# Priceincoding/nebula

Hardware: AMD Instinct MI355X
Metric: GTEPS for GO 3 STEPS on RMAT-26 at 1/2/4/8 GPUs; % of HBM roofline (higher is better)
Workload: dtype int64; 1 GPU; GO 3 STEPS FROM 64 seeds OVER follow WHERE follow.weight > 499 YIELD DISTINCT follow._dst; RMAT-26 ef16; vertices=32803048, edges_after_collapse=1060378721, edges_scanned_per_query=1545132647, parallelism=1 GPU

## Files before the change

nebula_amd/csrc/snapshot.hip:

```cpp
#include <climits>

#include <rocprim/device/device_merge.hpp>
#include <rocprim/device/device_radix_sort.hpp>
#include <rocprim/device/device_reduce.hpp>
#include <rocprim/device/device_scan.hpp>
#include <rocprim/device/device_select.hpp>
#include <rocprim/iterator/counting_iterator.hpp>

#include <algorithm>
#include <numeric>

#include "device_common.h"
#include "engine.h"
#include "qpred.h"
#include "query_common.h"

namespace nbg {

constexpr int kMaxFields = 64;
struct SchemaDev {
  int32_t nfields;
  int32_t types[kMaxFields];
};

// ... 1283 lines not shown
    case 4: k_gather_w<int32_t><<<g, 256, 0, c.stream>>>(static_cast<const int32_t*>(in), perm, static_cast<int32_t*>(out), m); break;
    default: k_gather_w<int64_t><<<g, 256, 0, c.stream>>>(static_cast<const int64_t*>(in), perm, static_cast<int64_t*>(out), m);
  }
}
static bool copy_prop(const PropCol& p) {
  bool intlike = p.type == NBG_T_INT || p.type == NBG_T_VID || p.type == NBG_T_TIMESTAMP || p.type == NBG_T_BOOL;
  return intlike && !p.present.p;
}


__global__ void k_live_bounds(const int64_t* trp, const uint32_t* odeg, int64_t n, unsigned long long* out) {
  unsigned long long a = 0, b = 0;
  for (int64_t i = blockIdx.x * int64_t(blockDim.x) + threadIdx.x; i < n; i += int64_t(gridDim.x) * blockDim.x)
    if (trp[i + 1] > trp[i]) {
      a = (unsigned long long)(i + 1);
      if (odeg[i]) b = (unsigned long long)(i + 1);
    }
  for (int o = 32; o > 0; o >>= 1) {
    a = max(a, (unsigned long long)__shfl_xor((long long)a, o));
    b = max(b, (unsigned long long)__shfl_xor((long long)b, o));
  }
  if ((threadIdx.x & 63) == 0) {
    if (a) atomicMax(out, a);
    if (b) atomicMax(out + 1, b);
  }
}
__global__ void k_odeg8(const uint32_t* deg, int64_t n, uint8_t* d8) {
  for (int64_t i = blockIdx.x * int64_t(blockDim.x) + threadIdx.x; i < n; i += int64_t(gridDim.x) * blockDim.x)
    d8[i] = uint8_t(min(deg[i], 255u));
}
__global__ void k_out_deg(const int64_t* row_ptr, const uint8_t* row_ok, int64_t n, uint32_t* deg,
                          unsigned int* maxd) {
  unsigned int m = 0;
  for (int64_t i = blockIdx.x * int64_t(blockDim.x) + threadIdx.x; i < n; i += int64_t(gridDim.x) * blockDim.x) {
    uint32_t d = uint32_t(row_ptr[i + 1] - row_ptr[i]);
    if (row_ok && !row_ok[i]) d = 0;
    deg[i] = d;
    m = d > m ? d : m;
  }
  if (maxd) atomicMax(maxd, m);
}
__global__ void k_hub_key(const int32_t* tsrc, int64_t m, const uint32_t* gdeg, uint32_t maxd, uint32_t* key) {
  for (int64_t i = blockIdx.x * int64_t(blockDim.x) + threadIdx.x; i < m; i += int64_t(gridDim.x) * blockDim.x)
    key[i] = maxd - gdeg[tsrc[i]];
}
__global__ void k_gather_u32(const uint32_t* in, const uint32_t* perm, uint32_t* out, int64_t m) {
  for (int64_t i = blockIdx.x * int64_t(blockDim.x) + threadIdx.x; i < m; i += int64_t(gridDim.x) * blockDim.x)
    out[i] = in[perm[i]];
}
__global__ void k_minmax_w(const void* data, int w, int64_t m, long long* mm) {
  long long lo = LLONG_MAX, hi = LLONG_MIN;
  for (int64_t i = blockIdx.x * int64_t(blockDim.x) + threadIdx.x; i < m; i += int64_t(gridDim.x) * blockDim.x) {
    long long v = w == 1 ? static_cast<const int8_t*>(data)[i]
                : w == 2 ? static_cast<const int16_t*>(data)[i]
                : w == 4 ? static_cast<const int32_t*>(data)[i]
                         : static_cast<const int64_t*>(data)[i];
    lo = v < lo ? v : lo;
    hi = v > hi ? v : hi;
  }
  for (int o = 32; o > 0; o >>= 1) {
    const long long a = __shfl_xor(lo, o), b = __shfl_xor(hi, o);
    lo = a < lo ? a : lo;
    hi = b > hi ? b : hi;
  }
  if ((threadIdx.x & 63) == 0) {
    atomicMin(mm, lo);
    atomicMax(mm + 1, hi);
  }
}
__global__ void k_pack_col(const int32_t* col, const void* data, int w, int64_t m, int64_t vmin, uint64_t range,
                           int gbits, int qbits, int32_t* out) {
  for (int64_t i = blockIdx.x * int64_t(blockDim.x) + threadIdx.x; i < m; i += int64_t(gridDim.x) * blockDim.x) {
    const int64_t v = w == 1 ? static_cast<const int8_t*>(data)[i]
                    : w == 2 ? static_cast<const int16_t*>(data)[i]
                    : w == 4 ? static_cast<const int32_t*>(data)[i]
                             : static_cast<const int64_t*>(data)[i];
    out[i] = int32_t((q_bucket(v, vmin, range, qbits) << gbits) | uint32_t(col[i]));
  }
}
template <typename T>
__global__ void k_build_pair(const int64_t* trp, const T* src, int64_t n, T* lo, T* hi, T none) {
  for (int64_t d = blockIdx.x * int64_t(blockDim.x) + threadIdx.x; d < n; d += int64_t(gridDim.x) * blockDim.x) {
    const int64_t b = trp[d], e = trp[d + 1];
#pragma unroll
    for (int q = 0; q < 4; q++) (q < 2 ? lo : hi)[size_t(d) * 2 + (q & 1)] = b + q < e ? src[b + q] : none;
  }
}

__global__ void k_tile_wide(const int64_t* trp, int64_t n, uint32_t* wide) {
  const int lane = threadIdx.x & 63;
  for (int64_t b = blockIdx.x * int64_t(blockDim.x) + threadIdx.x - lane; b < n; b += int64_t(gridDim.x) * blockDim.x) {
    const int64_t d = b + lane;
    const bool w = d < n && trp[d + 1] - trp[d] >= 3;
    const int64_t t = b >> 7;
    if (__ballot(w) != 0ull && lane == 0) atomicOr(wide + (t >> 5), 1u << (uint32_t(t) & 31u));
  }
}

__global__ void k_build_rec(const int64_t* trp, const int32_t* src, int64_t n, uint4* rec) {
  for (int64_t d = blockIdx.x * int64_t(blockDim.x) + threadIdx.x; d < n; d += int64_t(gridDim.x) * blockDim.x) {
    const int64_t b = trp[d], e = trp[d + 1];
    const uint64_t deg = uint64_t(e - b) < 65535u ? uint64_t(e - b) : 65535u;
    uint32_t w[16];
    w[0] = uint32_t(uint64_t(b));
    w[1] = uint32_t(uint64_t(b) >> 32) | uint32_t(deg << 16);
#pragma unroll
    for (int k = 0; k < kRecEntries; k++) w[2 + k] = b + k < e ? uint32_t(src[b + k]) : 0xffffffffu;
#pragma unroll
    for (int j = 0; j < 4; j++) rec[size_t(d) * 4 + j] = make_uint4(w[4 * j], w[4 * j + 1], w[4 * j + 2], w[4 * j + 3]);
  }
}

static void build_transpose(Ctx& c, EdgeSpace& es) {
  Csr& o = es.out;
  Csr& t = es.tr;
  const int64_t m = o.nnz;
  const int64_t lo = c.owned_lo(), hi = c.owned_hi();
  const int64_t n_own = hi - lo;
  const int G = c.world;
  auto nbits = [](int64_t x) {
    int b = 1;
    while ((int64_t(1) << b) < std::max<int64_t>(x, 2)) b++;
    return b;
  };
  const int64_t n_pad = (n_own + 127) / 128 * 128;
  es.odeg.alloc(size_t(n_pad + 1) * 4);
  NBG_HIP(hipMemsetAsync(es.odeg.p, 0, size_t(n_pad + 1) * 4, c.stream));
  DevBuf gdeg, dmax;
  dmax.alloc(16);
  NBG_HIP(hipMemsetAsync(dmax.p, 0, 16, c.stream));
  k_out_deg<<<grid_for(n_own), 256, 0, c.stream>>>(o.row_ptr.as<int64_t>(), o.row_ok.as<uint8_t>(), n_own,
                                                  es.odeg.as<uint32_t>(), dmax.as<unsigned int>());
  es.odeg8.alloc(size_t(n_pad + 64));
  k_odeg8<<<grid_for(n_pad + 1), 256, 0, c.stream>>>(es.odeg.as<uint32_t>(), n_pad + 1, es.odeg8.as<uint8_t>());
  const uint32_t* gdegp = es.odeg.as<uint32_t>();
  if (G > 1) {
    gdeg.alloc(size_t(c.n_global + 1) * 4);
    std::vector<size_t> rb(static_cast<size_t>(G)), ro(static_cast<size_t>(G));
    for (int p = 0; p < G; p++) {
      rb[size_t(p)] = size_t(c.base[size_t(p) + 1] - c.base[size_t(p)]) * 4;
      ro[size_t(p)] = size_t(c.base[size_t(p)]) * 4;
    }
    comm_allgatherv_bytes(c, es.odeg.p, size_t(n_own) * 4, gdeg.p, rb.data(), ro.data());
    gdegp = gdeg.as<uint32_t>();
  }
  uint32_t maxd = 0;
  NBG_HIP(hipMemcpyAsync(&maxd, dmax.p, 4, hipMemcpyDeviceToHost, c.stream));
  NBG_HIP(hipStreamSynchronize(c.stream));
  es.max_odeg = int64_t(maxd);
  if (G > 1) maxd = UINT32_MAX;
  DevBuf tdst, tsrc;
  int64_t R = 0;
  std::vector<const PropCol*> cp;
  for (const PropCol& p : o.props) cp.push_back(copy_prop(p) ? &p : nullptr);
  std::vector<DevBuf> rprops(o.props.size());
  {
    DevBuf esrc;
    esrc.alloc(size_t(m + 1) * 4);
    if (m) k_edge_src<<<grid_for(o.n_rows), 256, 0, c.stream>>>(o.row_ptr.as<int64_t>(), o.n_rows, esrc.as<int32_t>());
    if (G == 1) {
      R = m;
      tsrc = std::move(esrc);
      tdst.alloc(size_t(m + 1) * 4);
      if (m) NBG_HIP(hipMemcpyAsync(tdst.p, o.col.p, size_t(m) * 4, hipMemcpyDeviceToDevice, c.stream));
    } else {
      DevBuf keysB, iota, perm;
      keysB.alloc(size_t(m + 1) * 4);
      iota.alloc(size_t(m + 1) * 4);
      perm.alloc(size_t(m + 1) * 4);
      if (m) {
        k_iota_u32<<<grid_for(m), 256, 0, c.stream>>>(iota.as<uint32_t>(), m);
        radix_pairs<uint32_t, uint32_t>(c, o.col.as<uint32_t>(), keysB.as<uint32_t>(), iota.as<uint32_t>(),
                                       perm.as<uint32_t>(), m, nbits(c.n_global));
      }
      iota.release();
      DevBuf dbase, dcut;
      dbase.alloc(size_t(G + 1) * 8);
      dcut.alloc(size_t(G + 1) * 8);
// ... 57 lines not shown
  for (const PropCol& p : o.props) {
    PropCol q;
    q.name = p.name;
    q.type = p.type;
    q.width = p.width;
    t.props.push_back(std::move(q));
  }
  t.row_ptr.alloc(size_t(t.n_rows + 1) * 8);
  t.col.alloc(size_t(R) * 4 + 64);
  DevBuf perm;
  perm.alloc(size_t(R + 1) * 4);
  if (R) {
    DevBuf key, keyS, iota, perm1;
    key.alloc(size_t(R) * 4);
    keyS.alloc(size_t(R) * 4);
    iota.alloc(size_t(R) * 4);
    perm1.alloc(size_t(R) * 4);
    k_hub_key<<<grid_for(R), 256, 0, c.stream>>>(tsrc.as<int32_t>(), R, gdegp, maxd, key.as<uint32_t>());
    k_iota_u32<<<grid_for(R), 256, 0, c.stream>>>(iota.as<uint32_t>(), R);
    radix_pairs<uint32_t, uint32_t>(c, key.as<uint32_t>(), keyS.as<uint32_t>(), iota.as<uint32_t>(),
                                   perm1.as<uint32_t>(), R, G > 1 ? 32 : nbits(int64_t(maxd) + 1));
    iota.release();
    k_gather_u32<<<grid_for(R), 256, 0, c.stream>>>(tdst.as<uint32_t>(), perm1.as<uint32_t>(), key.as<uint32_t>(), R);
    radix_pairs<uint32_t, uint32_t>(c, key.as<uint32_t>(), keyS.as<uint32_t>(), perm1.as<uint32_t>(),
                                   perm.as<uint32_t>(), R, nbits(n_own));
    k_gather_w<int32_t><<<grid_for(R), 256, 0, c.stream>>>(tsrc.as<int32_t>(), perm.as<uint32_t>(), t.col.as<int32_t>(), R);
    rowptr_from_sorted(c, keyS.as<uint32_t>(), R, t.n_rows, t.row_ptr.as<int64_t>());
  } else {
    NBG_HIP(hipMemsetAsync(t.row_ptr.p, 0, size_t(t.n_rows + 1) * 8, c.stream));
  }
  tsrc.release();
  tdst.release();
  for (size_t f = 0; f < o.props.size(); f++) {
    if (!cp[f]) continue;
    int w = cp[f]->width;
    t.props[f].data.alloc(size_t(R) * size_t(w) + 16);
    const void* src = G == 1 ? cp[f]->data.p : rprops[f].p;
    if (R) gather_width(c, src, perm.as<uint32_t>(), t.props[f].data.p, R, w);
    rprops[f].release();
  }
  if (G == 1) {
    es.t_eid = std::move(perm);
    es.has_t_eid = true;
  } else {
    es.has_t_eid = false;
  }
  for (int h = 0; h < 2; h++) es.pair_col[h].release();
  es.tile_wide.release();
  es.q_field = -1;
  es.q_gbits = es.q_bits = 0;
  es.tcol_q.release();
  if (R > 0) {
    int gb = 1;
    while ((int64_t(1) << gb) <= c.n_global) gb++;
    const int qb = std::min(8, 31 - gb);
    int f = -1;
    for (size_t i = 0; i < t.props.size() && f < 0; i++)
      if (t.props[i].data.p) f = int(i);
    if (qb >= 3 && f >= 0) {
      const PropCol& pc = t.props[size_t(f)];
      DevBuf mm;
      mm.alloc(16);
      const long long init[2] = {LLONG_MAX, LLONG_MIN};
      NBG_HIP(hipMemcpyAsync(mm.p, init, 16, hipMemcpyHostToDevice, c.stream));
      k_minmax_w<<<grid_for(R), 256, 0, c.stream>>>(pc.data.p, pc.width, R, mm.as<long long>());
      long long h[2];
      NBG_HIP(hipMemcpyAsync(h, mm.p, 16, hipMemcpyDeviceToHost, c.stream));
      NBG_HIP(hipStreamSynchronize(c.stream));
      es.q_field = f;
      es.q_gbits = gb;
      es.q_bits = qb;
      es.q_min = h[0];
      es.q_range = uint64_t(h[1]) - uint64_t(h[0]) + 1;
      es.tcol_q.alloc(size_t(R) * 4 + 64);
      k_pack_col<<<grid_for(R), 256, 0, c.stream>>>(t.col.as<int32_t>(), pc.data.p, pc.width, R, es.q_min, es.q_range,
                                                   gb, qb, es.tcol_q.as<int32_t>());
      NBG_HIP(hipGetLastError());
    }
  }
  {
    const int64_t n_pad = (n_own + 127) / 128 * 128;
    for (int h = 0; h < 2; h++) {
      es.pair_col[h].alloc(size_t(n_pad) * 8 + 16);
      NBG_HIP(hipMemsetAsync(es.pair_col[h].as<uint8_t>() + size_t(n_own) * 8, 0xff, size_t(n_pad - n_own) * 8 + 16,
                             c.stream));
    }
    const int32_t* src_col = es.q_field >= 0 ? es.tcol_q.as<int32_t>() : t.col.as<int32_t>();
    if (n_own)
      k_build_pair<int32_t><<<grid_for(n_own), 256, 0, c.stream>>>(t.row_ptr.as<int64_t>(), src_col, n_own,
                                                                   es.pair_col[0].as<int32_t>(),
                                                                   es.pair_col[1].as<int32_t>(), -1);
    const int64_t nt = n_pad / 128;
    es.tile_wide.alloc(size_t(nt / 32 + 2) * 4);
    NBG_HIP(hipMemsetAsync(es.tile_wide.p, 0, size_t(nt / 32 + 2) * 4, c.stream));
    if (n_own)
      k_tile_wide<<<grid_for(n_own), 256, 0, c.stream>>>(t.row_ptr.as<int64_t>(), n_own, es.tile_wide.as<uint32_t>());
  }
  {
    DevBuf lb;
    lb.alloc(16);
    NBG_HIP(hipMemsetAsync(lb.p, 0, 16, c.stream));
    if (n_own)
      k_live_bounds<<<grid_for(n_own), 256, 0, c.stream>>>(t.row_ptr.as<int64_t>(), es.odeg.as<uint32_t>(), n_own,
                                                           lb.as<unsigned long long>());
    unsigned long long h[2] = {0, 0};
    NBG_HIP(hipMemcpyAsync(h, lb.p, 16, hipMemcpyDeviceToHost, c.stream));
    NBG_HIP(hipStreamSynchronize(c.stream));
    es.bu_in_tiles = int64_t((h[0] + 127) / 128);
    es.bu_both_tiles = int64_t((h[1] + 127) / 128);
  }
  es.brec.release();
  es.brec_rows = 0;
  {
    const int64_t rows = std::min(n_own, es.bu_in_tiles * 128);
    const int64_t cap_mb = c.opt("bu_rec_mb", 8192);
    if (rows > 0 && c.opt("bu_rec", 1) != 0 && rows * 64 <= (cap_mb << 20)) {
      es.brec.alloc(size_t(rows) * 64);
      const int32_t* src_col = es.q_field >= 0 ? es.tcol_q.as<int32_t>() : t.col.as<int32_t>();
      k_build_rec<<<grid_for(rows), 256, 0, c.stream>>>(t.row_ptr.as<int64_t>(), src_col, rows, es.brec.as<uint4>());
      NBG_HIP(hipGetLastError());
      es.brec_rows = rows;
    }
  }
  NBG_HIP(hipStreamSynchronize(c.stream));
  NBG_HIP(hipGetLastError());
  es.has_tr = true;
}

__global__ void k_owned_only(const uint64_t* in, int64_t n, int parts, int world, int rank, uint8_t* flag) {
  for (int64_t i = blockIdx.x * int64_t(blockDim.x) + threadIdx.x; i < n; i += int64_t(gridDim.x) * blockDim.x) {
    int64_t v = int64_t(in[i] ^ (1ull << 63));
    flag[i] = dev_owner(v, parts, world) == rank;
  }
}

__global__ void k_count_deg(const int64_t* src, int64_t n, const int64_t* keys, const int32_t* vals, uint64_t mask,
                            bool has_min, int32_t min_idx, unsigned int* deg) {
  for (int64_t i = blockIdx.x * int64_t(blockDim.x) + threadIdx.x; i < n; i += int64_t(gridDim.x) * blockDim.x) {
    const int32_t g = ht_lookup(keys, vals, mask, src[i], has_min, min_idx);
    if (g >= 0) atomicAdd(deg + g, 1u);
  }
}
__global__ void k_class_key(const unsigned int* odeg, const unsigned int* ideg, const uint32_t* idx, int64_t n,
                            uint64_t* key) {
  for (int64_t i = blockIdx.x * int64_t(blockDim.x) + threadIdx.x; i < n; i += int64_t(gridDim.x) * blockDim.x) {
    const int64_t u = idx ? int64_t(idx[i]) : i;
    const uint32_t od = odeg[u];
    if (ideg) {
      const uint32_t id = ideg[u];
      const uint64_t cls = id ? (od ? 0 : 1) : (od ? 2 : 3);
      key[i] = (cls << 34) | (uint64_t(~od) << 2) | uint64_t(3u - min(id, 3u));
    } else {
      key[i] = uint64_t(~od);
    }
  }
}

static void order_by_degree(Ctx& c, DevBuf& owned, int64_t n_owned) {
  if (n_owned <= 1) return;
  int64_t cap = 1024;
  while (cap < 2 * n_owned) cap <<= 1;
  DevBuf keys, vals, vids, deg, dmin;
  keys.alloc(size_t(cap) * 8);
  vals.alloc(size_t(cap) * 4);
  vids.alloc(size_t(n_owned) * 8);
  deg.alloc(size_t(n_owned) * 4);
  dmin.alloc(4);
  fill<int64_t>(c, keys.as<int64_t>(), INT64_MIN, cap);
  int32_t neg = -1;
  NBG_HIP(hipMemcpyAsync(dmin.p, &neg, 4, hipMemcpyHostToDevice, c.stream));
  NBG_HIP(hipMemsetAsync(deg.p, 0, size_t(n_owned) * 4, c.stream));
  k_unflip<<<grid_for(n_owned), 256, 0, c.stream>>>(owned.as<uint64_t>(), vids.as<int64_t>(), n_owned);
  k_ht_insert<<<grid_for(n_owned), 256, 0, c.stream>>>(keys.as<int64_t>(), vals.as<int32_t>(), uint64_t(cap - 1),
                                                       vids.as<int64_t>(), n_owned, 0, dmin.as<int32_t>());
  int32_t min_idx = -1;
  NBG_HIP(hipMemcpyAsync(&min_idx, dmin.p, 4, hipMemcpyDeviceToHost, c.stream));
  NBG_HIP(hipStreamSynchronize(c.stream));
// ... 1078 lines not shown
```

nebula_amd/csrc/traverse.hip:

```cpp
#include <chrono>
#include <rocprim/device/device_radix_sort.hpp>
#include <rocprim/device/device_reduce.hpp>
#include <rocprim/device/device_scan.hpp>
#include <rocprim/device/device_select.hpp>

#include <algorithm>
#include <cmath>
#include <unordered_map>
#include <thread>
#include <type_traits>
#include <initializer_list>

#include "device_common.h"
#include "engine.h"
#include "expr_device.h"
#include "program.h"
#include "qpred.h"
#include "query_common.h"
#include "rows.h"

namespace nbg {

constexpr int kThreads = 256;
constexpr int kItems = 8;
// ... 453 lines not shown
  }
}

struct GateIn {
  const unsigned long long* e = nullptr;
  const unsigned long long* n = nullptr;
  const unsigned long long* pg = nullptr;
  unsigned long long thr = 0;
  const unsigned long long* all = nullptr;
  int world = 1;
  int shards = 1;
};
__device__ inline bool gate_open(const GateIn& gi, unsigned long long* gate) {
  if (gi.e == nullptr && gi.all == nullptr) return gate == nullptr || *gate != 0ull;
  unsigned long long n, e;
  if (gi.all) {
    n = e = 0ull;
    for (int r = 0; r < gi.world; r++) n += gi.all[2 * r], e += gi.all[2 * r + 1];
  } else {
    n = e = 0ull;
    for (int s = 0; s < gi.shards; s++) n += gi.n[size_t(s) * kShardStride], e += gi.e[size_t(s) * kShardStride];
  }
  const bool open = (gi.pg == nullptr || *gi.pg != 0ull) && n > 0ull && e >= gi.thr;
  if (blockIdx.x == 0 && threadIdx.x == 0) {
    __hip_atomic_store(gate, open ? 1ull : 0ull, __ATOMIC_RELAXED, __HIP_MEMORY_SCOPE_AGENT);
    if (gi.all) {
      __hip_atomic_store(gate + (kSpecSumN - kSpecGate), n, __ATOMIC_RELAXED, __HIP_MEMORY_SCOPE_AGENT);
      __hip_atomic_store(gate + (kSpecSumE - kSpecGate), e, __ATOMIC_RELAXED, __HIP_MEMORY_SCOPE_AGENT);
    }
  }
  return open;
}

template <int PK, int U, int HUB, int STATS, int NT = 0, int SKIP = 0>
__global__ __launch_bounds__(1024, 8) void k_bu_lean(const uint2* __restrict__ lo, const uint2* __restrict__ hi,
                                                     int64_t ntiles, int64_t work_tiles,
                                                     const uint32_t* __restrict__ fbits, uint32_t fb_bytes,
                                                     unsigned long long* __restrict__ nbits,
                                                     unsigned long long* __restrict__ pbits,
                                                     const uint32_t* __restrict__ odeg, QArgs q_arg,
                                                     unsigned long long* __restrict__ partials, int cw,
                                                     const uint8_t* __restrict__ odeg8,
                                                     unsigned long long* gate, GateIn gi, int atomic_sums) {
  if (!gate_open(gi, gate)) return;
  __shared__ unsigned long long lds[kSlots * 16];
  extern __shared__ uint32_t s_fb[];
  if (HUB) hub_fill(s_fb, fbits, cw, true);
  const QArgs q = q_sgpr(q_arg);
  constexpr bool FINAL = PK == PK_FAST;
  constexpr int NS = FINAL ? 4 : 2;
  const __amdgpu_buffer_rsrc_t fb_rs =
      __builtin_amdgcn_make_buffer_rsrc(const_cast<uint32_t*>(fbits), 0, int(fb_bytes), 0x00020000);
  const uint32_t gmask = q.gmask, ucw = uint32_t(cw);
  const int lane = threadIdx.x & 63;
  const int64_t wave = (int64_t(blockIdx.x) * blockDim.x + threadIdx.x) >> 6;
  const int64_t nwaves = (int64_t(gridDim.x) * blockDim.x) >> 6;
  uint32_t nglob = 0, nhub = 0;
  unsigned long long nfound = 0, npend = 0, nwords = 0;
  unsigned long long odsum = 0;
  auto prep = [&](uint32_t sw, int k, uint32_t& goff, uint32_t& lidx, uint32_t& pm, uint32_t& um) {
    const uint32_t wi = (sw & gmask) >> 5;
    bool cand = true;
    if (FINAL) {
      const int st = q_test(int32_t(sw), q);
      const bool und = st < 0, pass = st > 0;
      cand = st != 0;
      pm |= pass ? 1u << k : 0u;
      um |= und ? 1u << k : 0u;
    }
    const bool hub = HUB && wi < ucw;
    goff = cand && !hub ? wi * 4u : 0xfffffff0u;
    lidx = cand && hub ? wi : ucw;
    if (STATS) {
      nglob += cand && !hub;
      nhub += cand && hub;
    }
  };
  auto bit = [](uint32_t w, uint32_t sw) -> uint32_t { return __builtin_amdgcn_ubfe(w, sw & 31u, 1u); };
  auto row_of = [&](int64_t t, int h) -> int64_t { return t * 128 + lane + 64 * h; };
  for (int64_t t0 = wave * U; t0 < work_tiles; t0 += nwaves * U) {
    uint2 a[U][2], b[U][2];
    uint32_t od[U][2];
    bool v[U];
#pragma unroll
    for (int u = 0; u < U; u++) {
      v[u] = t0 + u < work_tiles;
      const int64_t r = (v[u] ? t0 + u : t0) * 128 + lane;
#pragma unroll
      for (int h = 0; h < 2; h++) {
        if (NT) {
          const uint64_t x = __builtin_nontemporal_load(reinterpret_cast<const uint64_t*>(lo + r + 64 * h));
          a[u][h] = make_uint2(uint32_t(x), uint32_t(x >> 32));
          if (FINAL) {
            const uint64_t y = __builtin_nontemporal_load(reinterpret_cast<const uint64_t*>(hi + r + 64 * h));
            b[u][h] = make_uint2(uint32_t(y), uint32_t(y >> 32));
          }
          od[u][h] = FINAL ? 1u : uint32_t(__builtin_nontemporal_load(odeg8 + r + 64 * h));
        } else {
          a[u][h] = lo[r + 64 * h];
          if (FINAL) b[u][h] = hi[r + 64 * h];
          od[u][h] = FINAL ? 1u : odeg[r + 64 * h];
        }
      }
    }
    __builtin_amdgcn_sched_barrier(0);
    uint32_t goff[U][2][NS], lidx[U][2][NS], pm[U][2], um[U][2];
#pragma unroll
    for (int u = 0; u < U; u++)
#pragma unroll
      for (int h = 0; h < 2; h++) {
        pm[u][h] = um[u][h] = 0u;
        prep(a[u][h].x, 0, goff[u][h][0], lidx[u][h][0], pm[u][h], um[u][h]);
        prep(a[u][h].y, 1, goff[u][h][1], lidx[u][h][1], pm[u][h], um[u][h]);
        if (FINAL) {
          prep(b[u][h].x, 2, goff[u][h][2], lidx[u][h][2], pm[u][h], um[u][h]);
          prep(b[u][h].y, 3, goff[u][h][3], lidx[u][h][3], pm[u][h], um[u][h]);
        }
      }
    uint32_t lw[U][2][NS], gw[U][2][NS];
    if (HUB) {
#pragma unroll
      for (int u = 0; u < U; u++)
#pragma unroll
        for (int h = 0; h < 2; h++)
#pragma unroll
          for (int k = 0; k < NS; k++) {
            if (SKIP) {
              lw[u][h][k] = 0u;
              if (__ballot(lidx[u][h][k] != ucw)) lw[u][h][k] = s_fb[lidx[u][h][k]];
            } else {
              lw[u][h][k] = s_fb[lidx[u][h][k]];
            }
          }
    }
    bool noprobe[U][2];
#pragma unroll
    for (int u = 0; u < U; u++)
#pragma unroll
      for (int h = 0; h < 2; h++) {
        noprobe[u][h] = false;
        if ((SKIP & 2) && HUB && !FINAL) {
          const uint32_t sw[2] = {a[u][h].x, a[u][h].y};
          bool hf = false;
#pragma unroll
          for (int k = 0; k < NS; k++) hf = hf || bit(lw[u][h][k], sw[k]) != 0u;
          noprobe[u][h] = hf || od[u][h] == 0u;
        }
      }
#pragma unroll
    for (int u = 0; u < U; u++)
#pragma unroll
      for (int h = 0; h < 2; h++)
#pragma unroll
        for (int k = 0; k < NS; k++) {
          if (SKIP) {
            gw[u][h][k] = 0u;
            const uint32_t go = noprobe[u][h] ? 0xfffffff0u : goff[u][h][k];
            if (__ballot(go != 0xfffffff0u)) gw[u][h][k] = __builtin_amdgcn_raw_buffer_load_b32(fb_rs, go, 0, 0);
          } else {
            gw[u][h][k] = __builtin_amdgcn_raw_buffer_load_b32(fb_rs, goff[u][h][k], 0, 0);
          }
        }
    __builtin_amdgcn_sched_barrier(0);
    bool f[U][2], pend[U][2];
#pragma unroll
    for (int u = 0; u < U; u++) {
#pragma unroll
      for (int h = 0; h < 2; h++) {
        const uint32_t sw[4] = {a[u][h].x, a[u][h].y, b[u][h].x, b[u][h].y};
        uint32_t hm = 0u;
#pragma unroll
        for (int k = 0; k < NS; k++) hm |= bit(HUB ? (lw[u][h][k] | gw[u][h][k]) : gw[u][h][k], sw[k]) << k;
        if (FINAL) {
          f[u][h] = (hm & pm[u][h]) != 0u;
          pend[u][h] = v[u] && !f[u][h] && (b[u][h].y != 0xffffffffu || (hm & um[u][h]) != 0u);
        } else {
          f[u][h] = hm != 0u && od[u][h] > 0;
          pend[u][h] = v[u] && hm == 0u && od[u][h] > 0 && a[u][h].y != 0xffffffffu;
        }
      }
      nwords += v[u] ? (FINAL ? 8u : 4u) * 64u : 0u;
    }
    if (!FINAL) {
      bool anyp = false;
#pragma unroll
// ... 20 lines not shown
            prep(b[u][h].x, 0, g2[u][h][0], l2[u][h][0], d0, d1);
            prep(b[u][h].y, 1, g2[u][h][1], l2[u][h][1], d0, d1);
          }
        uint32_t lv[U][2][2], gv[U][2][2];
        if (HUB) {
#pragma unroll
          for (int u = 0; u < U; u++)
#pragma unroll
            for (int h = 0; h < 2; h++)
#pragma unroll
              for (int k = 0; k < 2; k++) lv[u][h][k] = s_fb[l2[u][h][k]];
        }
#pragma unroll
        for (int u = 0; u < U; u++)
#pragma unroll
          for (int h = 0; h < 2; h++)
#pragma unroll
            for (int k = 0; k < 2; k++) gv[u][h][k] = __builtin_amdgcn_raw_buffer_load_b32(fb_rs, g2[u][h][k], 0, 0);
#pragma unroll
        for (int u = 0; u < U; u++)
#pragma unroll
          for (int h = 0; h < 2; h++) {
            const uint32_t w0 = HUB ? (lv[u][h][0] | gv[u][h][0]) : gv[u][h][0];
            const uint32_t w1 = HUB ? (lv[u][h][1] | gv[u][h][1]) : gv[u][h][1];
            const bool g = (bit(w0, b[u][h].x) | bit(w1, b[u][h].y)) != 0u;
            f[u][h] = f[u][h] || (pend[u][h] && g);
            pend[u][h] = pend[u][h] && !g && b[u][h].y != 0xffffffffu;
          }
      } else {
#pragma unroll
        for (int u = 0; u < U; u++) pend[u][0] = pend[u][1] = false;
      }
    }
#pragma unroll
    for (int u = 0; u < U; u++) {
      if (!v[u]) continue;
      const int64_t t = t0 + u;
      unsigned long long f0 = __ballot(f[u][0]), f1 = __ballot(f[u][1]);
      unsigned long long p0 = __ballot(pend[u][0]), p1 = __ballot(pend[u][1]);
      if (SKIP & 4) {
        if (lane < 2) {
          typedef unsigned long long u64x2 __attribute__((ext_vector_type(2)));
          u64x2 vv;
          vv.x = lane ? p0 : f0;
          vv.y = lane ? p1 : f1;
          *reinterpret_cast<u64x2*>((lane ? pbits : nbits) + 2 * t) = vv;
        }
      } else if (lane < 2) {
        nbits[2 * t + lane] = lane ? f1 : f0;
        pbits[2 * t + lane] = lane ? p1 : p0;
      }
      nfound += uint64_t(__popcll(f0) + __popcll(f1));
      npend += uint64_t(__popcll(p0) + __popcll(p1));
      if (!FINAL) {
#pragma unroll
        for (int h = 0; h < 2; h++) {
          uint32_t d = f[u][h] ? od[u][h] : 0u;
          if (NT && d == 255u) d = odeg[row_of(t, h)];
          odsum += uint64_t(d);
        }
      }
    }
  }
  for (int64_t t = work_tiles + wave; t < ntiles; t += nwaves)
    if (lane < 2) {
      nbits[2 * t + lane] = 0ull;
      pbits[2 * t + lane] = 0ull;
    }
  if (lane != 0) nfound = npend = nwords = 0;
  unsigned long long acc64[8] = {nfound, odsum, nwords, npend, 0, 0, nglob, nhub};
  if (atomic_sums) block_add_sums(acc64, 8, lds, partials, atomic_sums);
  else block_store_partials(acc64, 8, lds, partials);
}

constexpr uint32_t kNoProbe = 0x0ffffff0u;
template <int CLS, int NT>
__global__ __launch_bounds__(1024, 8) void k_bu_fin(const uint2* __restrict__ lo, const uint2* __restrict__ hi,
                                                    int64_t ntiles, int64_t work_tiles,
                                                    const uint32_t* __restrict__ fbits,
                                                    unsigned long long* __restrict__ nbits,
                                                    unsigned long long* __restrict__ pbits, FinArgs fa_arg,
                                                    unsigned long long* __restrict__ partials, int cw,
                                                    uint32_t fb_rest, unsigned long long* gate, GateIn gi,
                                                    int atomic_sums, const uint32_t* __restrict__ wide) {
  if (!gate_open(gi, gate)) return;
  extern __shared__ uint32_t s_fb[];
  unsigned long long* lds = reinterpret_cast<unsigned long long*>(s_fb + ((cw + 2) & ~1));
  hub_fill(s_fb, fbits, cw, true);
  const uint32_t clo = __builtin_amdgcn_readfirstlane(fa_arg.clo), cr = __builtin_amdgcn_readfirstlane(fa_arg.cr);
  const uint32_t plo = __builtin_amdgcn_readfirstlane(fa_arg.plo), pr = __builtin_amdgcn_readfirstlane(fa_arg.pr);
  const bool pinv = __builtin_amdgcn_readfirstlane(fa_arg.pinv) != 0;
  const uint32_t bmask = __builtin_amdgcn_readfirstlane(fa_arg.bmask);
  const uint32_t cw4 = __builtin_amdgcn_readfirstlane(uint32_t(cw) * 4u);
  const __amdgpu_buffer_rsrc_t fb_rs = __builtin_amdgcn_make_buffer_rsrc(
      const_cast<uint32_t*>(fbits + cw), 0, int(__builtin_amdgcn_readfirstlane(fb_rest)), 0x00020000);
  typedef const __attribute__((address_space(3))) uint32_t* lds_u32p;
  const int lane = threadIdx.x & 63;
  const int64_t wave =
      int64_t(__builtin_amdgcn_readfirstlane(uint32_t((int64_t(blockIdx.x) * blockDim.x + threadIdx.x) >> 6)));
  const int64_t nwaves = (int64_t(gridDim.x) * blockDim.x) >> 6;
  unsigned long long nfound = 0, npend = 0, nwords = 0;
  auto ld8 = [&](const uint2* p) -> uint2 {
    if (!NT) return *p;
    const uint64_t x = __builtin_nontemporal_load(reinterpret_cast<const uint64_t*>(p));
    return make_uint2(uint32_t(x), uint32_t(x >> 32));
  };
  const uint32_t rest_b = __builtin_amdgcn_readfirstlane(fb_rest);
  auto tile = [&](int64_t t, auto ns_c) {
    constexpr int NS = decltype(ns_c)::value;
    uint32_t sw[2][NS];
    const int64_t r = t * 128 + lane;
#pragma unroll
    for (int h = 0; h < 2; h++) {
      const uint2 a = ld8(lo + r + 64 * h);
      sw[h][0] = a.x, sw[h][1] = a.y;
      if (NS == 4) {
        const uint2 b = ld8(hi + r + 64 * h);
        sw[h][NS - 2] = b.x, sw[h][NS - 1] = b.y;
      }
    }
    __builtin_amdgcn_sched_barrier(0);
    uint32_t ob[2][NS];
#pragma unroll
    for (int h = 0; h < 2; h++)
#pragma unroll
      for (int k = 0; k < NS; k++) {
        const uint32_t w = sw[h][k];
        if (CLS == 1)
          ob[h][k] = ((w >> 3) & bmask) | fin_skip_cls1(w, clo);
        else
          ob[h][k] = fin_candidate(w, clo, cr) ? (w >> 3) & bmask : kNoProbe;
      }
    uint32_t lw[2][NS], gw[2][NS];
#pragma unroll
    for (int h = 0; h < 2; h++)
#pragma unroll
      for (int k = 0; k < NS; k++) lw[h][k] = *(lds_u32p)(size_t(min(ob[h][k], cw4)));
    bool hubf[2] = {false, false};
#pragma unroll
    for (int h = 0; h < 2; h++)
#pragma unroll
      for (int k = 0; k < NS; k++) {
        const uint32_t w = sw[h][k];
        const bool pass = CLS == 1 ? w >= plo : (w - plo <= pr) != pinv;
        hubf[h] = hubf[h] || (__builtin_amdgcn_ubfe(lw[h][k], w, 1u) != 0u && pass);
      }
#pragma unroll
    for (int h = 0; h < 2; h++)
#pragma unroll
      for (int k = 0; k < NS; k++) {
        gw[h][k] = 0u;
        if (__ballot(ob[h][k] - cw4 < rest_b && !hubf[h]))
          gw[h][k] = __builtin_amdgcn_raw_buffer_load_b32(fb_rs, hubf[h] ? 0xfffffff0u : ob[h][k] - cw4, 0, 0);
      }
    __builtin_amdgcn_sched_barrier(0);
    bool f[2], pend[2];
#pragma unroll
    for (int h = 0; h < 2; h++) {
      bool fh = false, ah = false;
#pragma unroll
      for (int k = 0; k < NS; k++) {
        const uint32_t w = sw[h][k];
        const bool hit = __builtin_amdgcn_ubfe(lw[h][k] | gw[h][k], w, 1u) != 0u;
        const bool pass = CLS == 1 ? w >= plo : (w - plo <= pr) != pinv;
        fh = fh || (hit && pass);
        ah = ah || hit;
      }
      f[h] = fh;
      pend[h] = !fh && (ah || (NS == 4 && sw[h][NS - 1] != 0xffffffffu));
    }
    unsigned long long f0 = __ballot(f[0]), f1 = __ballot(f[1]);
    unsigned long long p0 = __ballot(pend[0]), p1 = __ballot(pend[1]);
    if (lane < 2) {
      typedef unsigned long long u64x2 __attribute__((ext_vector_type(2)));
      u64x2 v;
      v.x = lane ? p0 : f0;
      v.y = lane ? p1 : f1;
      *reinterpret_cast<u64x2*>((lane ? pbits : nbits) + 2 * t) = v;
    }
    nfound += uint64_t(__popcll(f0) + __popcll(f1));
    npend += uint64_t(__popcll(p0) + __popcll(p1));
    nwords += uint64_t(2 * NS) * 64u;
  };
  auto wide_word = [&](int64_t t) -> uint32_t {
    if (!wide) return 0xffffffffu;
    return wide[__builtin_amdgcn_readfirstlane(uint32_t(min(t, work_tiles) >> 5))];
  };
  uint32_t ww = wave < work_tiles ? wide_word(wave) : 0u;
  for (int64_t t = wave; t < work_tiles; t += nwaves) {
    const uint32_t wbit = __builtin_amdgcn_readfirstlane((ww >> (uint32_t(t) & 31u)) & 1u);
    __builtin_amdgcn_sched_barrier(0);
    ww = wide_word(t + nwaves);
    if (wbit)
      tile(t, std::integral_constant<int, 4>{});
    else
      tile(t, std::integral_constant<int, 2>{});
  }
  for (int64_t t = work_tiles + wave; t < ntiles; t += nwaves)
    if (lane < 2) {
      nbits[2 * t + lane] = 0ull;
      pbits[2 * t + lane] = 0ull;
    }
  if (lane != 0) nfound = npend = nwords = 0;
  unsigned long long acc64[8] = {nfound, 0, nwords, npend, 0, 0, 0, 0};
  if (atomic_sums) block_add_sums(acc64, 8, lds, partials, atomic_sums);
  else block_store_partials(acc64, 8, lds, partials);
}

constexpr int kLeanChunk = 8;
__device__ inline void load_chunk8(const int32_t* __restrict__ tcol, int64_t a, int64_t re, bool act,
                                   int32_t (&sv)[kLeanChunk]) {
  int4 x = make_int4(-1, -1, -1, -1), y = x;
  if (act) x = *reinterpret_cast<const int4*>(tcol + a);
  if (act && a + 4 < re) y = *reinterpret_cast<const int4*>(tcol + a + 4);
  sv[0] = x.x, sv[1] = x.y, sv[2] = x.z, sv[3] = x.w;
  sv[4] = y.x, sv[5] = y.y, sv[6] = y.z, sv[7] = y.w;
}
template <int PK, int W, int HUB, int REC>
__global__ __launch_bounds__(1024, 4) void k_bu_rest_lean(const unsigned long long* __restrict__ pbits, int64_t n,
                                                          const int64_t* __restrict__ trp,
                                                          const int32_t* __restrict__ tcol,
                                                          const uint32_t* __restrict__ fbits, uint32_t fb_bytes,
                                                          unsigned long long* nbits,
                                                          const uint32_t* __restrict__ odeg, FastArgs fp, QArgs q_arg,
                                                          unsigned long long* partials, int cw, int ru, int rest_from,
                                                          int steps, unsigned long long* dbg,
                                                          const unsigned long long* __restrict__ gate,
                                                          const uint4* __restrict__ rec, int atomic_sums) {
  if (gate && *gate == 0ull) return;
  const QArgs q = q_sgpr(q_arg);
  __shared__ unsigned long long lds[kSlots * 16];
  __shared__ unsigned long long s_found[16][64];
  extern __shared__ uint32_t s_fb[];
  const unsigned long long t_in = wall_clock64();
  if (HUB) hub_fill(s_fb, fbits, cw, false);
  const unsigned long long t_hub = wall_clock64();
  uint32_t d_rows = 0, d_batches = 0, d_steps = 0, d_scan = 0;
  unsigned long long t_scan = 0;
  const __amdgpu_buffer_rsrc_t fb_rs = __builtin_amdgcn_make_buffer_rsrc(
      const_cast<uint32_t*>(fbits), 0, int(__builtin_amdgcn_readfirstlane(fb_bytes)), 0x00020000);
  auto in_front = [&](int32_t g) -> bool {
    const int32_t wi = g >> 5;
    uint32_t w;
    if (HUB && wi < cw) w = s_fb[wi];
    else w = __builtin_amdgcn_raw_buffer_load_b32(fb_rs, wi * 4, 0, 0);
    return (w >> (g & 31)) & 1u;
  };
  uint32_t acc[6] = {0, 0, 0, 0, 0, 0};
  unsigned long long odsum = 0;
  const int lane = threadIdx.x & 63, wv = threadIdx.x >> 6;
  const int64_t nwords = (n + 63) / 64;
  const int64_t wave = (int64_t(blockIdx.x) * blockDim.x + threadIdx.x) >> 6;
  const int64_t nwaves = (int64_t(gridDim.x) * blockDim.x) >> 6;
  for (int64_t cbase = 0; cbase + wave < nwords; cbase += nwaves * 64) {
    const int64_t myw = cbase + int64_t(lane) * nwaves + wave;
    const unsigned long long pw = myw < nwords ? pbits[myw] : 0ull;
    s_found[wv][lane] = 0ull;
    uint32_t total;
    const uint32_t pre = wave_excl_scan(uint32_t(__popcll(pw)), total);
    for (uint32_t k0 = 0; k0 < total; k0 += 64) {
      const uint32_t p = k0 + uint32_t(lane);
      bool pend[1] = {p < total}, found[1] = {false};
      int64_t rb[1] = {0}, re[1] = {0};
      int wsel = 0;
#pragma unroll
      for (int st = 32; st > 0; st >>= 1) {
        const uint32_t pv = __shfl(pre, wsel + st);
        if (wsel + st < 64 && pv <= p) wsel += st;
      }
      const unsigned long long wbits = __shfl((long long)pw, wsel);
      const uint32_t kk = p - __shfl(pre, wsel);
      int bit = 0;
#pragma unroll
      for (int st = 32; st > 0; st >>= 1)
        if (uint32_t(__popcll(wbits & ((1ull << (bit + st)) - 1ull))) <= kk) bit += st;
      const int32_t r = int32_t((cbase + int64_t(wsel) * nwaves + wave) * 64 + bit);
      auto test_chunk = [&](const int32_t(&sv)[kLeanChunk], int64_t base, int64_t lo_e, int64_t hi_e, bool act,
                            bool count) __attribute__((always_inline)) -> bool {
        uint32_t w[kLeanChunk];
// ... 1165 lines not shown
}

static void launch_bits_vids(Ctx& c, const uint32_t* bits, int64_t rows, int64_t lo, void* out,
                             unsigned long long* n_out, const unsigned long long* gate) {
  const int grid = grid_cap((rows + 31) / 32, 1024, 4096);
  k_bits_compact<1, 8, 1><<<grid, 1024, 0, c.stream>>>(bits, rows, lo, c.vid_of.as<int64_t>(), out, n_out, gate);
}

struct BuLaunch {
  size_t ev_first = kNoEvent;
  std::string k0, k1;
  bool rest_rec = false;
  uint64_t od_bytes = 0;
  uint64_t flag_bytes = 0;
};
BuLaunch launch_bu_lean(Ctx& c, EdgeSpace& es, const uint32_t* fb, uint32_t* nbits, const uint32_t* odeg, int pk,
                      const FastArgs& fp, int fcol, unsigned long long* out, bool hop_front,
                      unsigned long long* gate = nullptr, GateIn gi = GateIn{}, bool out_zero = false,
                      int shards = 1) {
  const Csr& tr = es.tr;
  if (pk != PK_NONE && pk != PK_FAST) throw Error(NBG_E_DEVICE, "bottom-up hop with a VM predicate");
  if (!es.pair_col[0].p) throw Error(NBG_E_DEVICE, "bottom-up hop without the quad slab");
  const bool fast = pk == PK_FAST || !odeg;
  QArgs q;
  if (pk == PK_FAST) {
    q = make_qargs(es, c.opt("bu_qpred", 1) != 0 ? pk : PK_NONE, fcol, fp);
  } else {
    q = make_qargs(es, PK_NONE, -1, fp);
    if (fast) q.ulo = q.uhi = INT32_MAX, q.below = q.above = 1;
  }
  const int rest_from = pk == PK_FAST ? 0 : 4;
  pk = fast ? PK_FAST : PK_NONE;
  const int64_t ntiles = (tr.n_rows + 127) / 128;
  const int64_t work = std::min(ntiles, fast ? es.bu_in_tiles : es.bu_both_tiles);
  const int64_t waves = std::max<int64_t>(1, work);
  const int64_t fb_words = (c.n_global + 31) / 32;
  const int64_t hub_cap = std::max<int64_t>(0, c.opt("bu_hub_cap", 36 * 1024));
  const int cw = int(std::min<int64_t>(c.opt(fast ? "bu_lean_lds_kb_final" : "bu_lean_lds_kb", fast ? 72 : 64) * 256,
                                       std::min<int64_t>({fb_words, int64_t(36 * 1024), hub_cap})));
  const int bs = cw > 0 ? 1024 : 256;
  const int grid = int(std::max<int64_t>(
      1, std::min<int64_t>((waves + bs / 64 - 1) / (bs / 64),
                           std::min<int64_t>(cw > 0 ? 512 : 2048, kAggBlocks / 2))));
  const size_t shm = size_t(cw + 1) * 4;
  uint32_t fb_bytes = uint32_t(fb_words * 4);
  if (hop_front && !c.sharded && es.bu_both_tiles > 0)
    fb_bytes = uint32_t(std::min<int64_t>(fb_bytes, (es.bu_both_tiles * 128 + 31) / 32 * 4));
  const int probe_stats = int(c.opt("bu_probe_stats", 0));
  c.ws_pend.ensure(size_t(ntiles * 2 + 2) * 8);
  unsigned long long* pbits = c.ws_pend.as<unsigned long long>();
  const int atomic_sums =
      c.opt("bu_atomic_sums", 1) != 0 && c.opt("bu_rest_dbg", 0) == 0 ? (out_zero ? std::max(shards, 1) : 1) : 0;
  unsigned long long* partials = atomic_sums ? out : c.ws_partials.as<unsigned long long>();
  if (atomic_sums && !out_zero) NBG_HIP(hipMemsetAsync(out, 0, 8 * 8, c.stream));
  auto* nb = reinterpret_cast<unsigned long long*>(nbits);
  const uint2* lo = es.pair_col[0].as<uint2>();
  const uint2* hi = es.pair_col[1].as<uint2>();
  const uint32_t* od = fast ? nullptr : odeg;
  auto go = [&](auto kern) {
    if (shm > 48 * 1024)
      lds_limit(reinterpret_cast<const void*>(kern), shm);
    kern<<<grid, bs, shm, c.stream>>>(lo, hi, ntiles, work, fb, fb_bytes, nb, pbits, od, q, partials, cw,
                                      es.odeg8.as<uint8_t>(), gate, gi, atomic_sums);
  };
  int sel = probe_stats ? 4 + (cw > 0 ? 1 : 0) : (cw > 0 ? 2 : 0);
  if (sel == 2 && (fast || es.odeg8.p)) sel = 8;
#define NBG_LEAN(PKV)                                \
  switch (sel) {                                     \
    case 8: go(k_bu_lean<PKV, 1, 1, 0, 1, 3>); break; \
    case 0: go(k_bu_lean<PKV, 1, 0, 0>); break;      \
    case 2: go(k_bu_lean<PKV, 1, 1, 0>); break;      \
    case 4: go(k_bu_lean<PKV, 1, 0, 1>); break;      \
    default: go(k_bu_lean<PKV, 1, 1, 1>); break;     \
  }
  const bool fin = fast && !probe_stats && c.opt("bu_fin", 1) != 0;
  uint64_t flag_bytes = 0;
  char fin_nm[64] = "";
  if (fin) {
    const FinArgs fa = fin_args(q);
    const bool cls1 = fin_cls1_ok(fa) && c.opt("bu_fin_cls", 1) != 0;
    const size_t fshm = size_t((cw + 2) & ~1) * 4 + size_t(kSlots) * 16 * 8;
    const uint32_t rest = fb_bytes > uint32_t(cw) * 4u ? fb_bytes - uint32_t(cw) * 4u : 0u;
    const int nt = int(c.opt("bu_fin_nt", 1) != 0);
    const uint32_t* wide = c.opt("bu_fin_narrow", 1) != 0 ? es.tile_wide.as<uint32_t>() : nullptr;
    if (wide) flag_bytes = uint64_t(work) / 8;
    auto gof = [&](auto kern) {
      if (fshm > 48 * 1024) lds_limit(reinterpret_cast<const void*>(kern), fshm);
      kern<<<grid, bs, fshm, c.stream>>>(lo, hi, ntiles, work, fb, nb, pbits, fa, partials, cw, rest, gate, gi,
                                         atomic_sums, wide);
    };
    switch ((cls1 ? 1 : 0) | nt << 1) {
      case 0: gof(k_bu_fin<0, 0>); break;
      case 1: gof(k_bu_fin<1, 0>); break;
      case 2: gof(k_bu_fin<0, 1>); break;
      default: gof(k_bu_fin<1, 1>); break;
    }
    snprintf(fin_nm, sizeof fin_nm, "nbg::k_bu_fin<%d, %d>", cls1 ? 1 : 0, nt);
  } else if (fast) {
    NBG_LEAN(PK_FAST)
  } else {
    NBG_LEAN(PK_NONE)
  }
#undef NBG_LEAN
  NBG_HIP(hipGetLastError());
  const size_t ev_first = timing_event(c);
  const int64_t* trp = tr.row_ptr.as<int64_t>();
  const int32_t* tc = q.gbits ? es.tcol_q.as<int32_t>() : tr.col.as<int32_t>();
  const int ru = int(std::max<int64_t>(1, std::min<int64_t>(c.opt("bu_unroll", 1), kRestMax)));
  const int grid2 = 512;
  const int W = fast ? int(fp.width) : 0;
  const int rcw = int(std::min<int64_t>(c.opt(fast ? "bu_rest_lds_kb_final" : "bu_rest_lds_kb", 0) * 256,
                                        std::min<int64_t>({fb_words, int64_t(36 * 1024), hub_cap})));
  const size_t rshm = size_t(std::max(rcw, 1)) * 4;
  const int rsteps = int(std::max<int64_t>(1, c.opt("bu_rest_steps", 4)));
  DevBuf dbg_buf;
  unsigned long long* dbg = nullptr;
  if (c.opt("bu_rest_dbg", 0)) {
    dbg_buf.alloc(size_t(grid2) * 16 * 64);
    NBG_HIP(hipMemsetAsync(dbg_buf.p, 0, size_t(grid2) * 16 * 64, c.stream));
    dbg = dbg_buf.as<unsigned long long>();
  }
  const int64_t rest_rows = std::min(tr.n_rows, work * 128);
  const bool use_rec = es.brec.p && es.brec_rows >= std::min(tr.n_rows, work * 128) && c.opt("bu_rec", 1) != 0;
  const uint4* rec = use_rec ? es.brec.as<uint4>() : nullptr;
  auto rest = [&](auto kern) {
    if (rshm > 48 * 1024)
      lds_limit(reinterpret_cast<const void*>(kern), rshm);
    kern<<<grid2, 1024, rshm, c.stream>>>(pbits, rest_rows, trp, tc, fb, fb_bytes, nb, odeg, fp, q,
                                          atomic_sums ? partials : partials + grid, rcw, ru, rest_from, rsteps, dbg,
                                          gate, rec, atomic_sums);
  };
#define NBG_REST(PKV, WV)                                                 \
  if (rcw > 0) {                                                          \
    if (use_rec) rest(k_bu_rest_lean<PKV, WV, 1, 1>);                     \
    else rest(k_bu_rest_lean<PKV, WV, 1, 0>);                             \
  } else {                                                                \
    if (use_rec) rest(k_bu_rest_lean<PKV, WV, 0, 1>);                     \
    else rest(k_bu_rest_lean<PKV, WV, 0, 0>);                             \
  }
  if (fast) {
    switch (W) {
      case 1: NBG_REST(PK_FAST, 1); break;
      case 2: NBG_REST(PK_FAST, 2); break;
      case 4: NBG_REST(PK_FAST, 4); break;
      default: NBG_REST(PK_FAST, 8); break;
    }
  } else {
    NBG_REST(PK_NONE, 0);
  }
#undef NBG_REST
  NBG_HIP(hipGetLastError());
  if (!atomic_sums) k_reduce_partials<<<1, 1024, 0, c.stream>>>(partials, grid + grid2, out, gate);
  NBG_HIP(hipGetLastError());
  if (dbg) {
    std::vector<unsigned long long> h(size_t(grid2) * 16 * 8);
    NBG_HIP(hipMemcpyAsync(h.data(), dbg, h.size() * 8, hipMemcpyDeviceToHost, c.stream));
    NBG_HIP(hipStreamSynchronize(c.stream));
    if (const char* fn = getenv("NBG_DBG_FILE")) {
      if (FILE* f = fopen(fn, "ab")) {
        const uint64_t hdr[2] = {uint64_t(pk), uint64_t(grid2) * 16};
        fwrite(hdr, 8, 2, f);
        fwrite(h.data(), 8, h.size(), f);
        fclose(f);
      }
    }
  }
  char nm[96];
  if (fin)
    snprintf(nm, sizeof nm, "%s", fin_nm);
  else
    snprintf(nm, sizeof nm, "nbg::k_bu_lean<%d, 1, %d, %d%s>", pk, cw > 0 ? 1 : 0, probe_stats ? 1 : 0,
             sel == 8 ? ", 1, 3" : ", 0, 0");
// ... 1263 lines not shown
```

Baseline: 4131 GTEPS.

## Interleave lo pair columns per tile and add single-slot tier for degree-1 tiles

Changes the lo pair-column layout so slot 0 of both half-tiles is contiguous and slot 1 sits 128 entries later. Tiles whose vertices all have degree at most 1 can then read only the first slot block. A second per-tile flag word (degree >= 2) is added to tile_wide, and the fin kernel dispatches to NS=1, 2 or 4 variants, with NS=1 as the new default. This is meant to cut HBM bytes scanned for low-degree tiles in the bottom-up final step. The cost is twice as much flag metadata, and the lean kernel's loads now use the new layout, which is a consistency risk.

```diff
diff --git a/nebula_amd/csrc/snapshot.hip b/nebula_amd/csrc/snapshot.hip
--- a/nebula_amd/csrc/snapshot.hip
+++ b/nebula_amd/csrc/snapshot.hip
@@ -1389,8 +1389,13 @@
 __global__ void k_build_pair(const int64_t* trp, const T* src, int64_t n, T* lo, T* hi, T none) {
   for (int64_t d = blockIdx.x * int64_t(blockDim.x) + threadIdx.x; d < n; d += int64_t(gridDim.x) * blockDim.x) {
     const int64_t b = trp[d], e = trp[d + 1];
+    const size_t p = size_t(d >> 7) * 256 + size_t(d & 63) * 2 + size_t((d >> 6) & 1);
 #pragma unroll
-    for (int q = 0; q < 4; q++) (q < 2 ? lo : hi)[size_t(d) * 2 + (q & 1)] = b + q < e ? src[b + q] : none;
+    for (int q = 0; q < 4; q++) {
+      const T x = b + q < e ? src[b + q] : none;
+      if (q < 2) lo[p + size_t(q) * 128] = x;
+      else hi[size_t(d) * 2 + (q & 1)] = x;
+    }
   }
 }
 
@@ -1398,9 +1403,13 @@
   const int lane = threadIdx.x & 63;
   for (int64_t b = blockIdx.x * int64_t(blockDim.x) + threadIdx.x - lane; b < n; b += int64_t(gridDim.x) * blockDim.x) {
     const int64_t d = b + lane;
-    const bool w = d < n && trp[d + 1] - trp[d] >= 3;
+    const int64_t deg = d < n ? trp[d + 1] - trp[d] : 0;
     const int64_t t = b >> 7;
-    if (__ballot(w) != 0ull && lane == 0) atomicOr(wide + (t >> 5), 1u << (uint32_t(t) & 31u));
+    const bool w3 = __ballot(deg >= 3) != 0ull, w2 = __ballot(deg >= 2) != 0ull;
+    if (lane == 0) {
+      if (w3) atomicOr(wide + 2 * (t >> 5), 1u << (uint32_t(t) & 31u));
+      if (w2) atomicOr(wide + 2 * (t >> 5) + 1, 1u << (uint32_t(t) & 31u));
+    }
   }
 }
 
@@ -1624,8 +1633,8 @@
     const int64_t n_pad = (n_own + 127) / 128 * 128;
     for (int h = 0; h < 2; h++) {
       es.pair_col[h].alloc(size_t(n_pad) * 8 + 16);
-      NBG_HIP(hipMemsetAsync(es.pair_col[h].as<uint8_t>() + size_t(n_own) * 8, 0xff, size_t(n_pad - n_own) * 8 + 16,
-                             c.stream));
+      const size_t from = h == 0 ? 0 : size_t(n_own) * 8;
+      NBG_HIP(hipMemsetAsync(es.pair_col[h].as<uint8_t>() + from, 0xff, size_t(n_pad) * 8 + 16 - from, c.stream));
     }
     const int32_t* src_col = es.q_field >= 0 ? es.tcol_q.as<int32_t>() : t.col.as<int32_t>();
     if (n_own)
@@ -1633,8 +1642,8 @@
                                                                    es.pair_col[0].as<int32_t>(),
                                                                    es.pair_col[1].as<int32_t>(), -1);
     const int64_t nt = n_pad / 128;
-    es.tile_wide.alloc(size_t(nt / 32 + 2) * 4);
-    NBG_HIP(hipMemsetAsync(es.tile_wide.p, 0, size_t(nt / 32 + 2) * 4, c.stream));
+    es.tile_wide.alloc(size_t(nt / 32 + 2) * 8);
+    NBG_HIP(hipMemsetAsync(es.tile_wide.p, 0, size_t(nt / 32 + 2) * 8, c.stream));
     if (n_own)
       k_tile_wide<<<grid_for(n_own), 256, 0, c.stream>>>(t.row_ptr.as<int64_t>(), n_own, es.tile_wide.as<uint32_t>());
   }
diff --git a/nebula_amd/csrc/traverse.hip b/nebula_amd/csrc/traverse.hip
--- a/nebula_amd/csrc/traverse.hip
+++ b/nebula_amd/csrc/traverse.hip
@@ -559,25 +559,23 @@
     uint2 a[U][2], b[U][2];
     uint32_t od[U][2];
     bool v[U];
+    auto ld8 = [&](const uint2* p) -> uint2 {
+      if (!NT) return *p;
+      const uint64_t x = __builtin_nontemporal_load(reinterpret_cast<const uint64_t*>(p));
+      return make_uint2(uint32_t(x), uint32_t(x >> 32));
+    };
 #pragma unroll
     for (int u = 0; u < U; u++) {
       v[u] = t0 + u < work_tiles;
       const int64_t r = (v[u] ? t0 + u : t0) * 128 + lane;
+      const uint2 s0 = ld8(lo + r), s1 = ld8(lo + r + 64);
+      a[u][0] = make_uint2(s0.x, s1.x);
+      a[u][1] = make_uint2(s0.y, s1.y);
 #pragma unroll
       for (int h = 0; h < 2; h++) {
-        if (NT) {
-          const uint64_t x = __builtin_nontemporal_load(reinterpret_cast<const uint64_t*>(lo + r + 64 * h));
-          a[u][h] = make_uint2(uint32_t(x), uint32_t(x >> 32));
-          if (FINAL) {
-            const uint64_t y = __builtin_nontemporal_load(reinterpret_cast<const uint64_t*>(hi + r + 64 * h));
-            b[u][h] = make_uint2(uint32_t(y), uint32_t(y >> 32));
-          }
-          od[u][h] = FINAL ? 1u : uint32_t(__builtin_nontemporal_load(odeg8 + r + 64 * h));
-        } else {
-          a[u][h] = lo[r + 64 * h];
-          if (FINAL) b[u][h] = hi[r + 64 * h];
-          od[u][h] = FINAL ? 1u : odeg[r + 64 * h];
-        }
+        if (FINAL) b[u][h] = ld8(hi + r + 64 * h);
+        if (NT) od[u][h] = FINAL ? 1u : uint32_t(__builtin_nontemporal_load(odeg8 + r + 64 * h));
+        else od[u][h] = FINAL ? 1u : odeg[r + 64 * h];
       }
     }
     __builtin_amdgcn_sched_barrier(0);
@@ -764,7 +762,8 @@
                                                     unsigned long long* __restrict__ pbits, FinArgs fa_arg,
                                                     unsigned long long* __restrict__ partials, int cw,
                                                     uint32_t fb_rest, unsigned long long* gate, GateIn gi,
-                                                    int atomic_sums, const uint32_t* __restrict__ wide) {
+                                                    int atomic_sums, const uint32_t* __restrict__ wide,
+                                                    int one_slot) {
   if (!gate_open(gi, gate)) return;
   extern __shared__ uint32_t s_fb[];
   unsigned long long* lds = reinterpret_cast<unsigned long long*>(s_fb + ((cw + 2) & ~1));
@@ -792,11 +791,15 @@
     constexpr int NS = decltype(ns_c)::value;
     uint32_t sw[2][NS];
     const int64_t r = t * 128 + lane;
-#pragma unroll
-    for (int h = 0; h < 2; h++) {
-      const uint2 a = ld8(lo + r + 64 * h);
-      sw[h][0] = a.x, sw[h][1] = a.y;
-      if (NS == 4) {
+    const uint2 a = ld8(lo + r);
+    sw[0][0] = a.x, sw[1][0] = a.y;
+    if constexpr (NS >= 2) {
+      const uint2 a1 = ld8(lo + r + 64);
+      sw[0][1] = a1.x, sw[1][1] = a1.y;
+    }
+    if constexpr (NS == 4) {
+#pragma unroll
+      for (int h = 0; h < 2; h++) {
         const uint2 b = ld8(hi + r + 64 * h);
         sw[h][NS - 2] = b.x, sw[h][NS - 1] = b.y;
       }
@@ -864,19 +867,23 @@
     npend += uint64_t(__popcll(p0) + __popcll(p1));
     nwords += uint64_t(2 * NS) * 64u;
   };
-  auto wide_word = [&](int64_t t) -> uint32_t {
-    if (!wide) return 0xffffffffu;
-    return wide[__builtin_amdgcn_readfirstlane(uint32_t(min(t, work_tiles) >> 5))];
+  const uint32_t two_or = one_slot ? 0u : 0xffffffffu;
+  auto wide_word = [&](int64_t t) -> uint2 {
+    if (!wide) return make_uint2(0xffffffffu, 0xffffffffu);
+    return reinterpret_cast<const uint2*>(wide)[__builtin_amdgcn_readfirstlane(uint32_t(min(t, work_tiles) >> 5))];
   };
-  uint32_t ww = wave < work_tiles ? wide_word(wave) : 0u;
+  uint2 ww = wave < work_tiles ? wide_word(wave) : make_uint2(0u, 0u);
   for (int64_t t = wave; t < work_tiles; t += nwaves) {
-    const uint32_t wbit = __builtin_amdgcn_readfirstlane((ww >> (uint32_t(t) & 31u)) & 1u);
+    const uint32_t wbit = __builtin_amdgcn_readfirstlane((ww.x >> (uint32_t(t) & 31u)) & 1u);
+    const uint32_t tbit = __builtin_amdgcn_readfirstlane(((ww.y | two_or) >> (uint32_t(t) & 31u)) & 1u);
     __builtin_amdgcn_sched_barrier(0);
     ww = wide_word(t + nwaves);
     if (wbit)
       tile(t, std::integral_constant<int, 4>{});
+    else if (tbit)
+      tile(t, std::integral_constant<int, 2>{});
     else
-      tile(t, std::integral_constant<int, 2>{});
+      tile(t, std::integral_constant<int, 1>{});
   }
   for (int64_t t = work_tiles + wave; t < ntiles; t += nwaves)
     if (lane < 2) {
@@ -2208,12 +2215,13 @@
     const size_t fshm = size_t((cw + 2) & ~1) * 4 + size_t(kSlots) * 16 * 8;
     const uint32_t rest = fb_bytes > uint32_t(cw) * 4u ? fb_bytes - uint32_t(cw) * 4u : 0u;
     const int nt = int(c.opt("bu_fin_nt", 1) != 0);
-    const uint32_t* wide = c.opt("bu_fin_narrow", 1) != 0 ? es.tile_wide.as<uint32_t>() : nullptr;
-    if (wide) flag_bytes = uint64_t(work) / 8;
+    const int64_t narrow = c.opt("bu_fin_narrow", 2);
+    const uint32_t* wide = narrow != 0 ? es.tile_wide.as<uint32_t>() : nullptr;
+    if (wide) flag_bytes = uint64_t(work) / 4;
     auto gof = [&](auto kern) {
       if (fshm > 48 * 1024) lds_limit(reinterpret_cast<const void*>(kern), fshm);
       kern<<<grid, bs, fshm, c.stream>>>(lo, hi, ntiles, work, fb, nb, pbits, fa, partials, cw, rest, gate, gi,
-                                         atomic_sums, wide);
+                                         atomic_sums, wide, int(narrow >= 2));
     };
     switch ((cls1 ? 1 : 0) | nt << 1) {
       case 0: gof(k_bu_fin<0, 0>); break;
```

Measured after the change: 4170 GTEPS, median of 6. Within noise of the previous version (+0.9%).
